# kharchenkolab/dropEst

Hardware: AMD Instinct MI355X
Metric: Mreads/s processed to final count matrix (higher is better)
Workload: dtype u64

## Files before the change

dropest_amd/csrc/context.h:

```cpp
#pragma once

#include <algorithm>
#include <chrono>
#include <condition_variable>
#include <functional>
#include <mutex>
#include <cstring>
#include <map>
#include <memory>
#include <string>
#include <thread>
#include <unordered_map>
#include <unordered_set>
#include <vector>

#include "../../include/dropest_amd.h"
#include "k_cbhash.h"
#include "k_collisions.h"
#include "k_merge.h"
#include "k_umi_directional.h"
#include "whitelist.h"
#include "k_misc.h"
#include "k_radix.h"
#include "k_ssort.h"
// ... 526 lines not shown
	u32 main_sort_passes = 0, main_sort_kind = 0;
	void scan_counts(const u32 *in, u32 *out, u32 n, u32 *total_out);
	dropest::DevBuf<u32> scan_chunk;
	void radix_sort(u64 *&keys, u32 *&vals, u64 *&keys_alt, u32 *&vals_alt, u32 n, u64 varying_mask, int val_bytes = 4,
	                const char *stat_prefix = nullptr);
	dropest::DevBuf<u64> ss_sample_a, ss_sample_b, ss_fine, ss_coarse;
	dropest::DevBuf<u32> ss_base1, ss_cnt2, ss_bucket_base, ss_bucket_cnt, ss_tmp, ss_n_loc, ss_prefix, ss_chunk, ss_big_list;
	struct RecvChunk { hipEvent_t ev; dropest::CbRanges rg; };
	std::vector<RecvChunk> recv_chunks;
	double hot_coverage = 0;
	dropest::DevBuf<u32> ss_cg_loc, ss_cg_cnt, ss_cg_prefix;
	bool cg_from_sort = false;
	dropest::DevBuf<u32> ss_cursors;
	bool ss_no_reserve = false;
	bool splitter_sort_reduce();
	void reduce_all();
	void reduce_molecules_to_cell_gene();
	void reduce_cell_gene_to_cells();
	void refresh_real_rows();
	void upload_whitelist();
	void search_merge_candidates(const std::vector<u32> &cells, const dropest::MergeUniverse &U, dropest::MergeSearch &S);
	void search_merge_candidates_host(const std::vector<u32> &cells, const dropest::MergeUniverse &U, dropest::MergeSearch &S);
	void build_merge_pairs(const std::vector<u32> &cells, dropest::MergeSearch &S);
	void decide_merge_targets(const dropest::MergeUniverse &U, dropest::MergeSearch &S, const std::vector<u32> &inter,
	                          std::vector<long> &targets, std::vector<u32> &target_ridx);
	std::vector<std::vector<u32>> replay_candidate_orders(const dropest::MergeUniverse &U, dropest::MergeSearch &S,
	                                                      const std::vector<u32> &need_order);
	std::vector<u32> pair_intersections(const std::vector<u32> &pair_base_cell, const std::vector<u32> &pair_cand_cell);
	void pair_intersections(const std::vector<u32> &pair_base_cell, const std::vector<u32> &pair_cand_cell, std::vector<u32> &inter);
	std::vector<double> poisson_expected_intersections(const std::vector<u32> &pair_base_cell, const std::vector<u32> &pair_cand_cell);
// ... 175 lines not shown
```

dropest_amd/csrc/dropest_amd.hip:

```cpp

#include "context.h"
extern "C" void dropest_bgzf_warm_up(void *stream);
#include "k_keyscatter.h"
#include "k_umidict.h"

#include <atomic>
#include <functional>
#include <map>
#include <mutex>

using namespace dropest;

static thread_local std::string g_last_error;

template <class F>
static dropest_status guarded(F &&f) {
	try {
		f();
		return DROPEST_OK;
	} catch (const InvalidError &e) { g_last_error = e.what(); return DROPEST_ERR_INVALID;
	} catch (const RangeError &e) { g_last_error = e.what(); return DROPEST_ERR_RANGE;
	} catch (const UnsupportedError &e) { g_last_error = e.what(); return DROPEST_ERR_UNSUPPORTED;
	} catch (const IoError &e) { g_last_error = e.what(); return DROPEST_ERR_IO;
	} catch (const DeviceError &e) { g_last_error = e.what(); return DROPEST_ERR_DEVICE;
// ... 885 lines not shown
	d_in.alloc(h.size()); d_out.alloc(h.size());
	HIP_CHECK(hipMemcpyAsync(d_in.p, h.data(), h.size() * 4, hipMemcpyHostToDevice, stream));
	hipLaunchKernelGGL(ss_lds_order_probe_kernel, dim3(1), dim3(64), 0, stream, d_in.p, rounds, d_out.p);
	HIP_CHECK(hipGetLastError());
	HIP_CHECK(hipMemcpyAsync(got.data(), d_out.p, got.size() * 4, hipMemcpyDeviceToHost, stream));
	HIP_CHECK(stream_wait(stream));
	bool ordered = true;
	for (u32 r = 0; r < rounds && ordered; ++r) {
		u32 seen[64] = {0};
		for (u32 l = 0; l < 64; ++l) { const u32 d = h[size_t(r) * 64 + l]; if (got[size_t(r) * 64 + l] != seen[d]) ordered = false; ++seen[d]; }
	}
	if (!ordered) fprintf(stderr, "[dropest_amd] device %d: LDS atomics of one instruction are not applied in lane order here; the finishing sort of the splitter sort ranks with ballots (slower, same results)\n", device);
	return known[device] = ordered;
}

bool dropest_ctx::splitter_sort_reduce() {
	const u32 n = u32(n_reads);
	const SsPlan plan = ss_plan(n_reads, chr_from_gene, layout.val_bytes);
	if (!plan.applicable) return false;
	const int tb = plan.tb, fb1 = plan.fb1, fb2 = plan.fb2;
	const bool wide = fb2 > 9;
	const u32 F1 = 1u << fb1, Ff = 1u << fb2, F2 = F1 * Ff;
	const int ms = layout.mark_shift, VB = layout.val_bytes;
	(void)tb;
	uint64_t os_max = plan.os;
	if (const char *e = getenv("DROPEST_SSORT_OS")) os_max = uint64_t(std::max(1, atoi(e)));
	const u32 os = u32(std::max<uint64_t>(1, std::min<uint64_t>(os_max, uint64_t(n) / (uint64_t(F2) * 2))));
	const u32 n_sample = F2 * os;
	const u64 order_mask = ~((1ull << ms) - 1ull);
	const u64 varying = (counters.key_or ^ counters.key_and) & order_mask;
// ... 11 lines not shown
	const int VB2 = rebase ? 0 : VB, ms2 = rebase ? 3 : ms;
	const u64 rebase_mask = rebase ? ~((1ull << layout.umi_bits) - 1ull) : 0ull;
	if (!in_l1) {
		ss_sample_a.ensure(n_sample); ss_sample_b.ensure(n_sample); ss_fine.ensure(F2); ss_coarse.ensure(F1);
		timed("ss_sample", double(n_sample) * 16, [&] {
			hipLaunchKernelGGL(ss_sample_kernel, dim3(div_up(n_sample, 256)), dim3(256), 0, stream, keys, n, ms, n_sample, ss_sample_a.p);
		});
		ss_splitters_from_sample(n_sample, os, Ff, F2, varying >> ms);
	}

	const u32 n_tiles = div_up(n, SS_TILE);
	u32 nblocks = std::min<u32>(n_tiles, 1024);
	const u32 tpb = div_up(n_tiles, nblocks);
	nblocks = div_up(n_tiles, tpb);
	const u32 parts = std::max<u32>(1, std::min<u32>(16, 2048 / F1));
	ss_bucket_base.ensure(F2); ss_bucket_cnt.ensure(F2); scalars.ensure(16);
	HIP_CHECK(hipMemsetAsync(scalars.p, 0, 16, stream));
	u32 max_cnt = 0;
	static const u32 SMALL_MAX = [] { const char *e = getenv("DROPEST_SS_SMALL_MAX"); return e && atoi(e) >= 256 && atoi(e) <= 2048 ? u32(atoi(e)) : 2048u; }();
	const bool atomic_rank = lds_atomics_lane_ordered(cfg.device, stream);
	ss_tmp.ensure(span * 2 + 2); ss_n_loc.ensure(F2); ss_prefix.ensure(F2); ss_chunk.ensure(1024);
	SsLocalArgs a{};
	a.keys = keys; a.vals = vals; a.bucket_base = ss_bucket_base.p; a.bucket_cnt = ss_bucket_cnt.p; a.n_buckets = F2; a.ms = ms2;
	if (rebase) { a.rebase_coarse = ss_coarse.p; a.rebase_mask = rebase_mask; a.rebase_div = Ff; }
	a.t_key = keys_alt; a.t_reads = ss_tmp.p; a.t_agg = ss_tmp.p + span; a.n_loc = ss_n_loc.p;
	if (const char *e = getenv("DROPEST_SS_DEBUG")) a.debug = u32(atoi(e));
	a.order_flag = scalars.p + 2;
	a.atomic_below = u32(ms2 + layout.umi_bits);
	if (const char *e = getenv("DROPEST_SS_ATOMIC_BELOW")) a.atomic_below = u32(atoi(e));
	a.cap = SMALL_MAX; a.skip_above = SMALL_MAX;
	const bool fused_cg_off = getenv("DROPEST_SS_NO_FUSED_CG") != nullptr;
	const bool fuse_cg = !fused_cg_off;
	cg_from_sort = false;
// ... 32 lines not shown
		if (!in_l1) timed(VB ? "ss_scatter:L1:key+1B" : "ss_scatter:L1:keys", double(n) * (8 + VB + 8 + VB2), [&] {
			auto go = [&](auto kernel) { hipLaunchKernelGGL(kernel, dim3(nblocks), dim3(SS_T), 0, stream, keys, vals, keys_alt, vals_alt, n, ms, fb1, ss_coarse.p, tpb, r1, rebase_mask); };
			if (rebase) { if (wide) go(ss_scatter_res_l1_kernel<1, 1024, true>); else if (fb1 <= 8 && !no256) go(ss_scatter_res_l1_kernel<1, 256, true>); else go(ss_scatter_res_l1_kernel<1, 512, true>); }
			else if (wide) { if (VB) go(ss_scatter_res_l1_kernel<1, 1024>); else go(ss_scatter_res_l1_kernel<0, 1024>); }
			else if (fb1 <= 8 && !no256) { if (VB) go(ss_scatter_res_l1_kernel<1, 256>); else go(ss_scatter_res_l1_kernel<0, 256>); }
			else { if (VB) go(ss_scatter_res_l1_kernel<1, 512>); else go(ss_scatter_res_l1_kernel<0, 512>); }
		});
		timed(VB2 ? "ss_scatter:L2:key+1B" : "ss_scatter:L2:keys", double(n) * 2 * (8 + VB2), [&] {
			auto go = [&](auto kernel) { hipLaunchKernelGGL(kernel, dim3(F1 * parts), dim3(SS_T), 0, stream, keys_alt, vals_alt, keys, vals, ms2, fb2, ss_fine.p, cur1, CS1, cap1, parts, r2,
			                                                 rebase ? ss_coarse.p : static_cast<const u64 *>(nullptr), rebase_mask); };
			if (wide) { if (VB2) go(ss_scatter_res_l2_kernel<1, 1024>); else go(ss_scatter_res_l2_kernel<0, 1024>); }
			else if (fb2 <= 8 && !no256) { if (VB2) go(ss_scatter_res_l2_kernel<1, 256>); else go(ss_scatter_res_l2_kernel<0, 256>); }
			else { if (VB2) go(ss_scatter_res_l2_kernel<1, 512>); else go(ss_scatter_res_l2_kernel<0, 512>); }
		});
		timed("ss_scan", double(F2) * 12, [&] {
			hipLaunchKernelGGL(ss_res_buckets_kernel, dim3(div_up(F2, 256)), dim3(256), 0, stream, cur2, F2, cap2, ss_bucket_base.p, ss_bucket_cnt.p, scalars.p);
		});
		launch_small();
		u32 head[4] = {0, 0, 0, 0};
		fetch(head, scalars.p, 16);
		max_cnt = head[0];
		if (head[3]) {
			stats["count:ss_reserve_overflow"].launches += 1;
			ss_no_reserve = true;
			build_keys(false);
			return splitter_sort_reduce();
		}
		if (max_cnt > SS_LOCAL_MAX) { build_keys(false, false); return false; }
	} else {
	rs_hist.ensure(size_t(F1) * nblocks); rs_row_total.ensure(1024); ss_base1.ensure(F1 + 1);
	timed("ss_hist:L1", double(n) * 8, [&] {
		if (wide) hipLaunchKernelGGL(ss_hist_l1_kernel<1024>, dim3(nblocks), dim3(SS_T), 0, stream, keys, n, ms, fb1, ss_coarse.p, tpb, rs_hist.p);
		else hipLaunchKernelGGL(ss_hist_l1_kernel<512>, dim3(nblocks), dim3(SS_T), 0, stream, keys, n, ms, fb1, ss_coarse.p, tpb, rs_hist.p);
	});
	timed("ss_scan", double(F1) * nblocks * 8, [&] {
		hipLaunchKernelGGL(rs_scan_rows_kernel, dim3(F1), dim3(256), 0, stream, rs_hist.p, nblocks, rs_row_total.p);
		if (wide) hipLaunchKernelGGL(ss_scan_totals_kernel<1024>, dim3(1), dim3(1024), 0, stream, rs_row_total.p, F1, n, ss_base1.p);
		else hipLaunchKernelGGL(ss_scan_totals_kernel<512>, dim3(1), dim3(512), 0, stream, rs_row_total.p, F1, n, ss_base1.p);
	});
	timed(VB ? "ss_scatter:L1:key+1B" : "ss_scatter:L1:keys", double(n) * 2 * (8 + VB), [&] {
		auto go = [&](auto kernel) { hipLaunchKernelGGL(kernel, dim3(nblocks), dim3(SS_T), 0, stream, keys, vals, keys_alt, vals_alt, n, ms, fb1, ss_coarse.p, tpb, rs_hist.p, ss_base1.p); };
		if (wide) { if (VB) go(ss_scatter_l1_kernel<1, 1024>); else go(ss_scatter_l1_kernel<0, 1024>); }
		else { if (VB) go(ss_scatter_l1_kernel<1, 512>); else go(ss_scatter_l1_kernel<0, 512>); }
	});

	ss_cnt2.ensure(size_t(F2) * parts);
	timed("ss_hist:L2", double(n) * 8, [&] {
		if (wide) hipLaunchKernelGGL(ss_hist_l2_kernel<1024>, dim3(F1 * parts), dim3(SS_T), 0, stream, keys_alt, ms, fb2, ss_fine.p, ss_base1.p, parts, ss_cnt2.p);
		else hipLaunchKernelGGL(ss_hist_l2_kernel<512>, dim3(F1 * parts), dim3(SS_T), 0, stream, keys_alt, ms, fb2, ss_fine.p, ss_base1.p, parts, ss_cnt2.p);
	});
	timed("ss_scan", double(F2) * parts * 8, [&] {
		if (wide) hipLaunchKernelGGL(ss_scan_seg_kernel<1024>, dim3(F1), dim3(1024), 0, stream, ss_cnt2.p, Ff, parts, ss_base1.p, ss_bucket_base.p, ss_bucket_cnt.p, scalars.p);
		else hipLaunchKernelGGL(ss_scan_seg_kernel<512>, dim3(F1), dim3(512), 0, stream, ss_cnt2.p, Ff, parts, ss_base1.p, ss_bucket_base.p, ss_bucket_cnt.p, scalars.p);
	});
	fetch(&max_cnt, scalars.p, 4);
	if (max_cnt > SS_LOCAL_MAX) return false;
	timed(VB ? "ss_scatter:L2:key+1B" : "ss_scatter:L2:keys", double(n) * 2 * (8 + VB), [&] {
		auto go = [&](auto kernel) { hipLaunchKernelGGL(kernel, dim3(F1 * parts), dim3(SS_T), 0, stream, keys_alt, vals_alt, keys, vals, ms, fb2, ss_fine.p, ss_base1.p, parts, ss_cnt2.p); };
		if (wide) { if (VB) go(ss_scatter_l2_kernel<1, 1024>); else go(ss_scatter_l2_kernel<0, 1024>); }
		else { if (VB) go(ss_scatter_l2_kernel<1, 512>); else go(ss_scatter_l2_kernel<0, 512>); }
	});
	}

	if (!reserve) launch_small();
	if (max_cnt > SMALL_MAX) {
		std::vector<u32> cnts(F2), medium, big;
		fetch(cnts.data(), ss_bucket_cnt.p, size_t(F2) * 4);
		for (u32 b = 0; b < F2; ++b) if (cnts[b] > SMALL_MAX) (cnts[b] <= 4096 ? medium : big).push_back(b);
		ss_big_list.ensure(medium.size() + big.size());
		if (!medium.empty()) HIP_CHECK(hipMemcpyAsync(ss_big_list.p, medium.data(), medium.size() * 4, hipMemcpyHostToDevice, stream));
		if (!big.empty()) HIP_CHECK(hipMemcpyAsync(ss_big_list.p + medium.size(), big.data(), big.size() * 4, hipMemcpyHostToDevice, stream));
		auto launch = [&](auto kernel, u32 threads, u32 cap, const u32 *list, size_t count) {
			SsLocalArgs g = a;
			g.big_list = list; g.cap = cap; g.skip_above = cap;
			const size_t lds = ss_local_lds_bytes(cap, int(threads));
			HIP_CHECK(hipFuncSetAttribute(reinterpret_cast<const void *>(kernel), hipFuncAttributeMaxDynamicSharedMemorySize, int(lds)));
			hipLaunchKernelGGL(kernel, dim3(u32(count)), dim3(threads), lds, stream, g);
		};
		timed("ss_local:big", 0, [&] {
			if (atomic_rank) {
				if (!medium.empty()) { if (VB2) launch(ss_local_big_kernel<256, 1, true>, 256, 4096, ss_big_list.p, medium.size()); else launch(ss_local_big_kernel<256, 0, true>, 256, 4096, ss_big_list.p, medium.size()); }
				if (!big.empty()) { if (VB2) launch(ss_local_big_kernel<512, 1, true>, 512, SS_LOCAL_MAX, ss_big_list.p + medium.size(), big.size()); else launch(ss_local_big_kernel<512, 0, true>, 512, SS_LOCAL_MAX, ss_big_list.p + medium.size(), big.size()); }
			} else {
				if (!medium.empty()) { if (VB2) launch(ss_local_big_kernel<256, 1>, 256, 4096, ss_big_list.p, medium.size()); else launch(ss_local_big_kernel<256, 0>, 256, 4096, ss_big_list.p, medium.size()); }
				if (!big.empty()) { if (VB2) launch(ss_local_big_kernel<512, 1>, 512, SS_LOCAL_MAX, ss_big_list.p + medium.size(), big.size()); else launch(ss_local_big_kernel<512, 0>, 512, SS_LOCAL_MAX, ss_big_list.p + medium.size(), big.size()); }
			}
		});
		HIP_CHECK(stream_wait(stream));
	}
	const u32 n_chunks = div_up(F2, 1024);
	timed("ss_scan", double(F2) * 12, [&] {
		hipLaunchKernelGGL(ss_chunk_sums_kernel<1024>, dim3(n_chunks), dim3(1024), 0, stream, ss_n_loc.p, F2, ss_chunk.p);
		hipLaunchKernelGGL(ss_prefix_kernel<1024>, dim3(n_chunks), dim3(1024), 0, stream, ss_n_loc.p, F2, ss_chunk.p, n_chunks, ss_prefix.p, scalars.p + 1);
		if (fuse_cg) {
			hipLaunchKernelGGL(ss_cg_counts_kernel, dim3(div_up(F2, 256)), dim3(256), 0, stream, ss_bucket_base.p, ss_n_loc.p, keys_alt, layout.umi_bits, F2, ss_cg_loc.p, ss_cg_cnt.p);
			hipLaunchKernelGGL(ss_chunk_sums_kernel<1024>, dim3(n_chunks), dim3(1024), 0, stream, ss_cg_cnt.p, F2, ss_chunk.p);
			hipLaunchKernelGGL(ss_prefix_kernel<1024>, dim3(n_chunks), dim3(1024), 0, stream, ss_cg_cnt.p, F2, ss_chunk.p, n_chunks, ss_cg_prefix.p, scalars.p + 4);
		}
	});
	u32 total_flag[4] = {0, 0, 0, 0};
	fetch(total_flag, scalars.p + 1, 16);
	if (total_flag[1]) {
		if (atomic_rank) lds_atomics_mark_unordered(cfg.device);
// ... 85 lines not shown
	const size_t quads = words / 4;
	for (uint32_t k = 0; k < a.n_arrays; ++k) {
		uint4 *q = reinterpret_cast<uint4 *>(a.p[k]);
		for (size_t i = size_t(blockIdx.x) * 256 + threadIdx.x; i < quads; i += size_t(gridDim.x) * 256) q[i] = make_uint4(0, 0, 0, 0);
		if (blockIdx.x == 0 && threadIdx.x < words - quads * 4) a.p[k][quads * 4 + threadIdx.x] = 0;
	}
}

void dropest_ctx::reduce_all() {
	const u32 n = u32(n_reads);
	u64 *keys = keys_a.p, *keys_alt = keys_b.p;
	u32 *vals = vals_a.p, *vals_alt = vals_b.p;
	const u64 order_mask = ~((1ull << layout.mark_shift) - 1ull);
	const u64 varying = (counters.key_or ^ counters.key_and) & order_mask;
	if (splitter_sort_reduce()) {
		n_chr_rows = 0;
		if (!cg_from_sort) reduce_molecules_to_cell_gene();
		reduce_cell_gene_to_cells();
		HIP_CHECK(stream_wait(stream));
		return;
	}
	main_sort_passes = u32(plan_radix_passes(varying).size()); main_sort_kind = 0;
	radix_sort(keys, vals, keys_alt, vals_alt, n, varying, layout.val_bytes);

	if (chr_from_gene) {
		auto run = [&](auto &p) {
			p.keys = keys;
			n_mol = run_segmented_reduce(*this, "molecules", p, n, 8 + layout.val_bytes, [&](u32 total) {
				mol_key.ensure(total + 1);
				for (DevBuf<u32> *b : {&mol_reads, &mol_mark, &mol_exon, &mol_intron}) b->ensure(total + 1);
// ... 1595 lines not shown
```

dropest_amd/csrc/k_misc.h:

```cpp
#pragma once

#include "k_cbhash.h"
#include "util.h"

namespace dropest {

__global__ __launch_bounds__(1024) void scan_small_kernel(const uint32_t *__restrict__ in, uint32_t *__restrict__ out,
                                                          uint32_t n, uint32_t *__restrict__ total_out) {
	__shared__ uint32_t scratch[1024 / 64 + 1];
	uint32_t carry = 0;
	for (uint32_t base = 0; base < n; base += 1024) {
		uint32_t i = base + threadIdx.x;
		uint32_t v = i < n ? in[i] : 0;
		uint32_t total;
		uint32_t ex = block_excl_scan_u32<1024>(v, scratch, total);
		if (i < n) out[i] = carry + ex;
		carry += total;
	}
	if (threadIdx.x == 0 && total_out) *total_out = carry;
}

struct KeyLayout {
	int umi_bits, gene_bits, cell_bits;
	int mark_shift;
// ... 292 lines not shown
				}
				if (t < total - tail0) { a.t_drow8[out + tail0 + t] = stage_d[tail0 + t]; a.t_val8[out + tail0 + t] = stage_v[tail0 + t]; }
			}
			if (threadIdx.x == 0 && total) kept_row[0] = kept_row[total];
		} else if (keep) {
			if (NARROW) {
				a.t_gene16[out + ex] = uint16_t(g);
				a.t_val16[out + ex] = v >= 0xFFFFu ? uint16_t(0xFFFFu) : uint16_t(v);
				if (v >= 0xFFFFu) {
					const uint32_t at = atomicAdd(a.ovf_count, 1u);
					if (at < a.ovf_cap) { a.ovf_pos[at] = out + ex; a.ovf_val[at] = v; }
				}
			} else { a.t_gene[out + ex] = g; a.t_val[out + ex] = v; }
		}
		out += total;
	}
}

constexpr uint32_t EMS_COLS = 8, EMS_STAGE = EMS_COLS * 255u;
__global__ __launch_bounds__(256) void emit_matrix_bytes_short_kernel(MatrixArgs a) {
	__shared__ uint32_t st_pos[2][EMS_STAGE], st_val[2][EMS_STAGE];
	__shared__ uint32_t st_n[2], st_base[2];
	const uint32_t lane = threadIdx.x & 63u, w = threadIdx.x >> 6;
	if (threadIdx.x < 2) st_n[threadIdx.x] = 0;
	__syncthreads();
	for (uint32_t c = w; c < EMS_COLS; c += 4) {
		const uint32_t idx = blockIdx.x * EMS_COLS + c;
		if (idx >= a.n_list) break;
		const uint32_t col = a.col_list[idx];
		const uint32_t cell = a.col_cell[col];
// ... 453 lines not shown
```

dropest_amd/csrc/k_ssort.h:

```cpp
#pragma once

#include "util.h"

namespace dropest {

constexpr int SS_T = 512, SS_I = 8, SS_TILE = SS_T * SS_I;
constexpr int SS_MAX_F = 512;
constexpr uint32_t SS_LOCAL_MAX = 8192;

__global__ __launch_bounds__(256) void ss_sample_kernel(const unsigned long long *__restrict__ keys, uint32_t n, int ms,
                                                        uint32_t n_sample, unsigned long long *__restrict__ out) {
	const uint32_t j = blockIdx.x * 256 + threadIdx.x;
	if (j >= n_sample) return;
	const uint32_t pos = uint32_t((uint64_t(j) * n + n / 2) / n_sample);
	out[j] = keys[pos < n ? pos : n - 1] >> ms;
}

__global__ __launch_bounds__(256) void ss_pick_splitters_kernel(const unsigned long long *__restrict__ sorted_sample, uint32_t os, uint32_t F, uint32_t F2,
                                                                unsigned long long *__restrict__ fine, unsigned long long *__restrict__ coarse) {
	const uint32_t j = blockIdx.x * 256 + threadIdx.x;
	if (j >= F2) return;
	const unsigned long long v = j + 1 < F2 ? sorted_sample[size_t(j + 1) * os] : ~0ull;
	fine[j] = v;
	if ((j + 1) % F == 0) coarse[(j + 1) / F - 1] = v;
// ... 65 lines not shown
__global__ __launch_bounds__(SS_T) void ss_hist_l2_kernel(const unsigned long long *__restrict__ keys, int ms, int fb,
                                                          const unsigned long long *__restrict__ fine, const uint32_t *__restrict__ base1,
                                                          uint32_t parts, uint32_t *__restrict__ cnt2) {
	__shared__ unsigned long long sp[MAXF];
	__shared__ uint32_t cnt[MAXF];
	const uint32_t F = 1u << fb, s = blockIdx.x / parts, p = blockIdx.x % parts;
	for (uint32_t j = threadIdx.x; j < F; j += SS_T) { sp[j] = j + 1 < F ? fine[size_t(s) * F + j] : ~0ull; cnt[j] = 0; }
	__syncthreads();
	uint32_t begin, end;
	ss_l2_range(base1, s, p, parts, begin, end);
	if (begin < end) ss_hist_range(keys, begin, end, ms, fb, sp, cnt);
	__syncthreads();
	for (uint32_t j = threadIdx.x; j < F; j += SS_T) cnt2[(size_t(s) * F + j) * parts + p] = cnt[j];
}

template <int MAXF>
__global__ __launch_bounds__(MAXF) void ss_scan_seg_kernel(uint32_t *__restrict__ cnt2, uint32_t F, uint32_t parts,
                                                            const uint32_t *__restrict__ base1, uint32_t *__restrict__ bucket_base,
                                                            uint32_t *__restrict__ bucket_cnt, uint32_t *__restrict__ max_cnt) {
	__shared__ uint32_t scratch[MAXF / 64 + 1];
	const uint32_t s = blockIdx.x, f = threadIdx.x;
	uint32_t *row = cnt2 + (size_t(s) * F + f) * parts;
	uint32_t sum = 0;
	if (f < F) for (uint32_t p = 0; p < parts; ++p) sum += row[p];
	uint32_t total;
	const uint32_t ex = block_excl_scan_u32<MAXF>(sum, scratch, total);
	if (f < F) {
		uint32_t run = base1[s] + ex;
		bucket_base[size_t(s) * F + f] = run;
		bucket_cnt[size_t(s) * F + f] = sum;
		for (uint32_t p = 0; p < parts; ++p) { const uint32_t c = row[p]; row[p] = run; run += c; }
	}
	const unsigned long long m = wave_reduce_max_u64(sum);
	if (lane_id() == 0 && m) atomicMax(max_cnt, uint32_t(m));
}

template <int VB, int MAXF>
__device__ inline void ss_scatter_range(const unsigned long long *__restrict__ keys, const uint8_t *__restrict__ vals,
                                        unsigned long long *__restrict__ okeys, uint8_t *__restrict__ ovals, uint32_t begin, uint32_t end,
                                        int ms, int fb, const unsigned long long *sp, uint32_t *goff, uint32_t *cnt, uint32_t *tstart,
                                        uint32_t *gdelta, uint32_t *scratch, unsigned long long *sk, uint16_t *sd, uint8_t *sv) {
	constexpr int PER = MAXF / SS_T;
	const uint32_t F = 1u << fb, tid = threadIdx.x;
	for (uint32_t t0 = begin; t0 < end; t0 += SS_TILE) {
		const uint32_t in_tile = end - t0 < uint32_t(SS_TILE) ? end - t0 : uint32_t(SS_TILE);
		for (uint32_t j = tid; j < F; j += SS_T) cnt[j] = 0;
		lds_barrier();
		unsigned long long key[SS_I];
		uint8_t val[VB ? SS_I : 1];
// ... 225 lines not shown
	const unsigned long long lo = (rebase_coarse && s) ? (rebase_coarse[s - 1] & rebase_mask) : 0ull;
	for (uint32_t j = threadIdx.x; j < F; j += SS_T) {
		const unsigned long long f = j + 1 < F ? fine[size_t(s) * F + j] : ~0ull;
		sp[j] = j + 1 < F ? (f > lo ? f - lo : 0ull) : ~0ull;
	}
	__syncthreads();
	const uint32_t fill = cur1[size_t(s) * cstride1], sb = s * cap1, se = sb + (fill < cap1 ? fill : cap1);
	const uint32_t tiles = (se - sb + SS_TILE - 1) / SS_TILE, tpp = (tiles + parts - 1) / parts;
	const uint64_t b = uint64_t(sb) + uint64_t(p) * tpp * SS_TILE, e = b + uint64_t(tpp) * SS_TILE;
	const uint32_t begin = b < se ? uint32_t(b) : se, end = e < se ? uint32_t(e) : se;
	SsReserve mine = rs;
	mine.first = s * F;
	if (begin < end) ss_scatter_res_range<VB, MAXF>(keys, vals, okeys, ovals, begin, end, ms, fb, sp, mine, cnt, tstart, gdelta, scratch, sk, sd, sv);
}
__global__ __launch_bounds__(256) void ss_res_buckets_kernel(const uint32_t *__restrict__ cur2, uint32_t n_buckets, uint32_t cap,
                                                             uint32_t *__restrict__ bucket_base, uint32_t *__restrict__ bucket_cnt, uint32_t *__restrict__ max_cnt) {
	const uint32_t b = blockIdx.x * 256 + threadIdx.x;
	uint32_t c = 0;
	if (b < n_buckets) { c = cur2[b] < cap ? cur2[b] : cap; bucket_base[b] = b * cap; bucket_cnt[b] = c; }
	const unsigned long long m = wave_reduce_max_u64(c);
	if (lane_id() == 0 && m) atomicMax(max_cnt, uint32_t(m));
}

struct SsLocalArgs {
	const unsigned long long *keys;
	const uint8_t *vals;
	const uint32_t *bucket_base, *bucket_cnt;
	const uint32_t *big_list;
	uint32_t n_buckets;
	int ms;
	uint32_t cap;
	uint32_t skip_above;
	uint32_t debug;
	uint32_t atomic_below;
	uint32_t *order_flag;
	unsigned long long *t_key;
	uint32_t *t_reads, *t_agg, *n_loc;
	uint32_t *cg_loc;
	int cg_shift;
	const unsigned long long *rebase_coarse;
	unsigned long long rebase_mask;
	uint32_t rebase_div;
};

template <int THREADS, int ITEMS, int VB, bool ATOMIC_RANK = false>
__device__ inline void ss_local_run(const SsLocalArgs &a, uint32_t bucket, uint32_t base, uint32_t cnt, unsigned char *smem) {
	constexpr uint32_t WAVES = THREADS / 64;
	const uint32_t tid = threadIdx.x, w = tid >> 6, lane = tid & 63u;
	unsigned long long *sk = reinterpret_cast<unsigned long long *>(smem);
	uint32_t *agg = reinterpret_cast<uint32_t *>(smem);
	uint32_t *headpos = agg + a.cap;
	uint32_t *wcnt = reinterpret_cast<uint32_t *>(smem + size_t(a.cap) * 8);
	uint32_t *tstart = wcnt + WAVES * 256;
	uint32_t *scratch = tstart + 256;
	uint32_t *wtot = scratch + (THREADS / 64 + 1);
	uint32_t *misc = wtot + WAVES;
	unsigned long long *red = reinterpret_cast<unsigned long long *>(misc + 4 + ((WAVES + 1) & 1u));
	uint8_t *sv = reinterpret_cast<uint8_t *>(red + 2 * WAVES);
	const int ms = a.ms;
	const uint32_t coarse_b = a.rebase_coarse ? bucket / a.rebase_div : 0u;
	const unsigned long long kbase = coarse_b ? (a.rebase_coarse[coarse_b - 1u] & a.rebase_mask) : 0ull;

	const uint32_t lane_off = w * (64 * ITEMS) + lane;
	unsigned long long key[ITEMS];
	uint8_t val[VB ? ITEMS : 1];
	unsigned long long k_or = 0, k_and = ~0ull;
#pragma unroll
	for (int i = 0; i < ITEMS; ++i) {
		const uint32_t p = lane_off + i * 64;
		const bool valid = p < cnt;
		key[i] = valid ? a.keys[base + p] : 0ull;
		if (VB) val[i] = valid ? a.vals[base + p] : uint8_t(0);
	}
#pragma unroll
	for (int i = 0; i < ITEMS; ++i) {
		const uint32_t p = lane_off + i * 64;
		if (p < cnt) { k_or |= key[i]; k_and &= key[i]; sk[p] = key[i]; if (VB) sv[p] = val[i]; }
	}
	k_or = wave_reduce_or_u64(k_or); k_and = wave_reduce_and_u64(k_and);
	if (lane == 0) { red[2 * w] = k_or; red[2 * w + 1] = k_and; }
	lds_barrier();
	k_or = 0; k_and = ~0ull;
#pragma unroll
	for (uint32_t k = 0; k < WAVES; ++k) { k_or |= red[2 * k]; k_and &= red[2 * k + 1]; }
	const unsigned long long vary = (k_or ^ k_and) & ~((1ull << ms) - 1ull);

	for (int shift = vary ? __builtin_ctzll(vary) : 64; shift < 64 && (vary >> shift) != 0; shift += 8) {
		if (((vary >> shift) & 0xFFull) == 0 || (a.debug & 2u)) continue;
		for (uint32_t j = tid; j < WAVES * 256; j += THREADS) wcnt[j] = 0;
		lds_barrier();
		uint32_t lrank[ITEMS];
		const bool by_atomic = ATOMIC_RANK && uint32_t(shift) < a.atomic_below;
		const uint32_t vbits = uint32_t(vary >> shift) & 0xFFu;
#pragma unroll
		for (int i = 0; i < ITEMS; ++i) {
			const bool valid = (lane_off + i * 64) < cnt;
			const uint32_t d = uint32_t(key[i] >> shift) & 0xFFu;
			if (by_atomic) { lrank[i] = valid ? atomicAdd(&wcnt[w * 256 + d], 1u) : 0u; continue; }
			uint32_t diff_lo = 0, diff_hi = 0;
			for (uint32_t left = vbits; left; left &= left - 1u) {
				const int b = __builtin_ctz(left);
				const int32_t mine = int32_t(d << (31 - b)) >> 31;
				const unsigned long long bal = __ballot(mine != 0);
				diff_lo |= uint32_t(bal) ^ uint32_t(mine);
				diff_hi |= uint32_t(bal >> 32) ^ uint32_t(mine);
			}
			unsigned long long m = ~(((unsigned long long)diff_hi << 32) | diff_lo);
			m &= __ballot(valid);
			const uint32_t before = __builtin_amdgcn_mbcnt_hi(uint32_t(m >> 32), __builtin_amdgcn_mbcnt_lo(uint32_t(m), 0u));
			const uint32_t old = wcnt[w * 256 + d];
// ... 19 lines not shown
			for (uint32_t j = 0; j < PER; ++j) {
				const uint32_t d = tid * PER + j;
				uint32_t run = 0;
#pragma unroll
				for (uint32_t k = 0; k < WAVES; ++k) { const uint32_t c = wcnt[k * 256 + d]; wcnt[k * 256 + d] = run; run += c; }
				tot[j] = run; sum += run;
			}
			uint32_t total;
			uint32_t ex = block_excl_scan_u32<THREADS, true>(sum, scratch, total);
#pragma unroll
			for (uint32_t j = 0; j < PER; ++j) { tstart[tid * PER + j] = ex; ex += tot[j]; }
		}
		lds_barrier();
#pragma unroll
		for (int i = 0; i < ITEMS; ++i)
			if ((lane_off + i * 64) < cnt) {
				const uint32_t d = uint32_t(key[i] >> shift) & 0xFFu;
				const uint32_t q = tstart[d] + wcnt[w * 256 + d] + lrank[i];
				sk[q] = key[i];
				if (VB) sv[q] = val[i];
			}
		lds_barrier();
#pragma unroll
		for (int i = 0; i < ITEMS; ++i) {
			const uint32_t p = lane_off + i * 64;
			if (p < cnt) { key[i] = sk[p]; if (VB) val[i] = sv[p]; }
		}
	}

	uint32_t run = 0, pre[ITEMS], head_bits = 0, cg_heads = 0;
	bool out_of_order = false;
#pragma unroll
	for (int i = 0; i < ITEMS; ++i) {
		const uint32_t p = lane_off + i * 64;
		const bool valid = p < cnt;
		const unsigned long long prev = (valid && p) ? sk[p - 1] : 0ull;
		out_of_order |= valid && p && (prev >> ms) > (key[i] >> ms);
		const bool head = valid && (p == 0 || (prev >> ms) != (key[i] >> ms));
		const unsigned long long bal = __ballot(head);
		pre[i] = run + __builtin_amdgcn_mbcnt_hi(uint32_t(bal >> 32), __builtin_amdgcn_mbcnt_lo(uint32_t(bal), 0u));
		run += uint32_t(__popcll(bal));
		if (head) head_bits |= 1u << i;
		if (a.cg_loc) cg_heads += uint32_t(__popcll(__ballot(valid && p && (prev >> a.cg_shift) != (key[i] >> a.cg_shift))));
	}
	if (lane == 0) wtot[w] = run;
	if (a.cg_loc && lane == 0 && cg_heads) atomicAdd(&a.cg_loc[bucket], cg_heads);
	if (__ballot(out_of_order) && lane == 0) atomicOr(a.order_flag, 1u);
	lds_barrier();
	uint32_t woff = 0, n_loc = 0;
#pragma unroll
	for (uint32_t k = 0; k < WAVES; ++k) { const uint32_t t = wtot[k]; if (k < w) woff += t; n_loc += t; }
	for (uint32_t m = tid; m < n_loc; m += THREADS) agg[m] = 0;
	if (tid == 0) a.n_loc[bucket] = n_loc;
	lds_barrier();
#pragma unroll
	for (int i = 0; i < ITEMS; ++i) {
		const uint32_t p = lane_off + i * 64;
		if (p >= cnt) continue;
		const uint32_t is_head = (head_bits >> i) & 1u;
		const uint32_t m = woff + pre[i] + is_head - 1u;
		const uint32_t mark = VB ? uint32_t(val[i]) & 7u : uint32_t(key[i]) & 7u;
		if (is_head) { headpos[m] = p; a.t_key[base + m] = (key[i] >> ms) + kbase; }
		const uint32_t add = (((mark >> 1) & 1u) << 1) | (((mark >> 2) & 1u) << 16);
		if (add) atomicAdd(&agg[m], add);
		if (mark & 1u) atomicOr(&agg[m], 1u);
	}
	lds_barrier();
	for (uint32_t m = tid; m < n_loc; m += THREADS) {
		const uint32_t e = m + 1 < n_loc ? headpos[m + 1] : cnt;
		a.t_reads[base + m] = e - headpos[m];
		a.t_agg[base + m] = agg[m];
	}
}

template <int VB, bool ATOMIC_RANK = false>
__global__ __launch_bounds__(256) void ss_local_kernel(SsLocalArgs a) {
	extern __shared__ __attribute__((aligned(16))) unsigned char ss_smem[];
	const uint32_t b = blockIdx.x;
	const uint32_t cnt = a.bucket_cnt[b], base = a.bucket_base[b];
	if (cnt == 0) { if (threadIdx.x == 0) a.n_loc[b] = 0; return; }
	if (cnt > a.skip_above) return;
	if (cnt <= 1024) ss_local_run<256, 4, VB, ATOMIC_RANK>(a, b, base, cnt, ss_smem);
	else ss_local_run<256, 8, VB, ATOMIC_RANK>(a, b, base, cnt, ss_smem);
}
template <int THREADS, int VB, bool ATOMIC_RANK = false>
__global__ __launch_bounds__(THREADS) void ss_local_wave_kernel(SsLocalArgs a) {
	extern __shared__ __attribute__((aligned(16))) unsigned char ss_smem[];
	const uint32_t b = blockIdx.x;
	const uint32_t cnt = a.bucket_cnt[b], base = a.bucket_base[b];
	if (cnt == 0) { if (threadIdx.x == 0) a.n_loc[b] = 0; return; }
	if (cnt > a.skip_above) return;
	if (cnt <= 1024) ss_local_run<THREADS, 1024 / THREADS, VB, ATOMIC_RANK>(a, b, base, cnt, ss_smem);
	else ss_local_run<THREADS, 2048 / THREADS, VB, ATOMIC_RANK>(a, b, base, cnt, ss_smem);
}
template <int THREADS, int VB, bool ATOMIC_RANK = false>
__global__ __launch_bounds__(THREADS) void ss_local_big_kernel(SsLocalArgs a) {
	extern __shared__ __attribute__((aligned(16))) unsigned char ss_smem[];
	const uint32_t b = a.big_list[blockIdx.x];
// ... 255 lines not shown
```

dropest_amd/csrc/matrix_emit.h:

```cpp
#pragma once

#include <sys/syscall.h>
#include <unistd.h>

static u32 checked_nnz(uint64_t nnz) {
	if (nnz > 0xFFFFFFF0ull) throw UnsupportedError("count matrix with more than 2^32 non-zeros");
	return u32(nnz);
}

void dropest_ctx::matrix_columns(bool filtered_m, std::vector<u32> &col_cell, std::vector<u32> &colptr, uint64_t &nnz) {
	col_cell.clear(); colptr.clear();
	nnz = 0;
	if (filtered_m) {
		filtered_cells();
		for (u32 ri : filtered_ridx) {
			const HostCell &h = real[ri];
			col_cell.push_back(h.id); colptr.push_back(u32(nnz)); nnz += h.row.requested_genes;
		}
	} else {
		constexpr unsigned W = dropest::HostPool::MAX;
		size_t cols[W] = {0}; uint64_t sums[W] = {0};
		auto is_col = [&](const HostCell &h) { return !(h.merged || h.excluded || h.row.n_genes < min_before); };
		const unsigned workers = parallel_ranges(real.size(), [&](size_t b, size_t e, unsigned w) {
			size_t c = 0; uint64_t s = 0;
// ... 58 lines not shown
}

void dropest_ctx::launch_emit(int dev_form, dropest::MatrixArgs a, MatrixResult &M, hipStream_t st) {
	using namespace dropest;
	const u32 ncols = u32(M.ncols);
	if (dev_form == 0) { hipLaunchKernelGGL(emit_matrix_kernel<0>, dim3(ncols), dim3(256), 0, st, a); return; }
	if (dev_form == 1) { hipLaunchKernelGGL(emit_matrix_kernel<1>, dim3(ncols), dim3(256), 0, st, a); return; }
	auto is_long = [&](u32 j) { return M.colptr[j + 1] - M.colptr[j] >= 256u; };
	M.col_list_host.resize(ncols);
	u32 n_long = 0;
	for (u32 j = 0; j < ncols; ++j) if (is_long(j)) M.col_list_host[n_long++] = j;
	u32 at = n_long;
	for (u32 j = 0; j < ncols; ++j) if (!is_long(j)) M.col_list_host[at++] = j;
	M.d_col_list.ensure(ncols);
	HIP_CHECK(hipMemcpyAsync(M.d_col_list.p, M.col_list_host.data(), size_t(ncols) * 4, hipMemcpyHostToDevice, st));
	if (n_long) { a.col_list = M.d_col_list.p; a.n_list = n_long; hipLaunchKernelGGL(emit_matrix_kernel<2>, dim3(n_long), dim3(256), 0, st, a); }
	if (ncols > n_long) {
		a.col_list = M.d_col_list.p + n_long; a.n_list = ncols - n_long;
		hipLaunchKernelGGL(emit_matrix_bytes_short_kernel, dim3(div_up(a.n_list, EMS_COLS)), dim3(256), 0, st, a);
	}
}

void dropest_ctx::matrix_copy_out(MatrixResult &M, uint64_t nnz, hipStream_t st) {
	if (M.narrow == 2) {
		HIP_CHECK(hipMemcpyAsync(M.h_drow8.p, M.d_drow8.p, nnz, hipMemcpyDeviceToHost, st));
		HIP_CHECK(hipMemcpyAsync(M.h_val8.p, M.d_val8.p, nnz, hipMemcpyDeviceToHost, st));
		HIP_CHECK(hipMemcpyAsync(M.vals.h_count(), M.vals.d_count(), 4, hipMemcpyDeviceToHost, st));
		HIP_CHECK(hipMemcpyAsync(M.rows.h_count(), M.rows.d_count(), 4, hipMemcpyDeviceToHost, st));
	} else if (M.narrow == 1) {
		HIP_CHECK(hipMemcpyAsync(M.h_row16.p, M.d_row16.p, nnz * 2, hipMemcpyDeviceToHost, st));
		HIP_CHECK(hipMemcpyAsync(M.h_val16.p, M.d_val16.p, nnz * 2, hipMemcpyDeviceToHost, st));
// ... 522 lines not shown
```

Baseline: 11200.

## Build oversize bucket lists on device, size local sort per bucket, add byte emit kernel

The scan kernels now classify oversize buckets into medium and big lists on the device with wave ballots and an atomic counter. This replaces the host fetch of all bucket counts, the host partitioning, the list upload and a stream wait. The local sort picks exact items-per-thread variants (5, 6, 7 or 8) and skips unused register slots when fewer items are needed. A new raw byte-packed emit kernel writes four delta and value bytes per thread for long columns when zeros are not skipped. Extra profiling statistics are added, and list ordering now depends on atomics, so the order of bucket processing may differ between runs.

```diff
diff --git a/dropest_amd/csrc/context.h b/dropest_amd/csrc/context.h
--- a/dropest_amd/csrc/context.h
+++ b/dropest_amd/csrc/context.h
@@ -564,6 +564,8 @@
 	dropest::DevBuf<u32> ss_cursors;
 	bool ss_no_reserve = false;
 	bool splitter_sort_reduce();
+	u32 ss_stat_buckets = 0, ss_stat_small_max = 0;
+	void ss_count_items_per_wave(u32 F2, u32 small_max);
 	void reduce_all();
 	void reduce_molecules_to_cell_gene();
 	void reduce_cell_gene_to_cells();
diff --git a/dropest_amd/csrc/dropest_amd.hip b/dropest_amd/csrc/dropest_amd.hip
--- a/dropest_amd/csrc/dropest_amd.hip
+++ b/dropest_amd/csrc/dropest_amd.hip
@@ -923,6 +923,14 @@
 	return known[device] = ordered;
 }
 
+void dropest_ctx::ss_count_items_per_wave(u32 F2, u32 small_max) {
+	std::vector<u32> cnts(F2);
+	fetch(cnts.data(), ss_bucket_cnt.p, size_t(F2) * 4);
+	u32 by_ipw[17] = {0};
+	for (u32 c : cnts) if (c && c <= SS_LOCAL_MAX) by_ipw[div_up(c, c <= small_max || c <= 4096u ? 256u : 512u)] += 1;
+	for (u32 k = 1; k <= 16; ++k) if (by_ipw[k]) stats["count:ss_local_ipw" + std::to_string(k)].launches += by_ipw[k];
+}
+
 bool dropest_ctx::splitter_sort_reduce() {
 	const u32 n = u32(n_reads);
 	const SsPlan plan = ss_plan(n_reads, chr_from_gene, layout.val_bytes);
@@ -964,9 +972,10 @@
 	const u32 tpb = div_up(n_tiles, nblocks);
 	nblocks = div_up(n_tiles, tpb);
 	const u32 parts = std::max<u32>(1, std::min<u32>(16, 2048 / F1));
-	ss_bucket_base.ensure(F2); ss_bucket_cnt.ensure(F2); scalars.ensure(16);
-	HIP_CHECK(hipMemsetAsync(scalars.p, 0, 16, stream));
-	u32 max_cnt = 0;
+	ss_bucket_base.ensure(F2); ss_bucket_cnt.ensure(F2); ss_big_list.ensure(F2); scalars.ensure(16);
+	HIP_CHECK(hipMemsetAsync(scalars.p, 0, 32, stream));
+	u32 max_cnt = 0, n_medium = 0, n_big = 0;
+	unsigned long long *const big_counts = reinterpret_cast<unsigned long long *>(scalars.p + 6);
 	static const u32 SMALL_MAX = [] { const char *e = getenv("DROPEST_SS_SMALL_MAX"); return e && atoi(e) >= 256 && atoi(e) <= 2048 ? u32(atoi(e)) : 2048u; }();
 	const bool atomic_rank = lds_atomics_lane_ordered(cfg.device, stream);
 	ss_tmp.ensure(span * 2 + 2); ss_n_loc.ensure(F2); ss_prefix.ensure(F2); ss_chunk.ensure(1024);
@@ -1029,12 +1038,13 @@
 			else { if (VB2) go(ss_scatter_res_l2_kernel<1, 512>); else go(ss_scatter_res_l2_kernel<0, 512>); }
 		});
 		timed("ss_scan", double(F2) * 12, [&] {
-			hipLaunchKernelGGL(ss_res_buckets_kernel, dim3(div_up(F2, 256)), dim3(256), 0, stream, cur2, F2, cap2, ss_bucket_base.p, ss_bucket_cnt.p, scalars.p);
+			hipLaunchKernelGGL(ss_res_buckets_kernel, dim3(div_up(F2, 256)), dim3(256), 0, stream, cur2, F2, cap2, ss_bucket_base.p, ss_bucket_cnt.p, scalars.p,
+			                   SMALL_MAX, ss_big_list.p, big_counts);
 		});
 		launch_small();
-		u32 head[4] = {0, 0, 0, 0};
-		fetch(head, scalars.p, 16);
-		max_cnt = head[0];
+		u32 head[8] = {0, 0, 0, 0, 0, 0, 0, 0};
+		fetch(head, scalars.p, 32);
+		max_cnt = head[0]; n_medium = head[6]; n_big = head[7];
 		if (head[3]) {
 			stats["count:ss_reserve_overflow"].launches += 1;
 			ss_no_reserve = true;
@@ -1065,10 +1075,14 @@
 		else hipLaunchKernelGGL(ss_hist_l2_kernel<512>, dim3(F1 * parts), dim3(SS_T), 0, stream, keys_alt, ms, fb2, ss_fine.p, ss_base1.p, parts, ss_cnt2.p);
 	});
 	timed("ss_scan", double(F2) * parts * 8, [&] {
-		if (wide) hipLaunchKernelGGL(ss_scan_seg_kernel<1024>, dim3(F1), dim3(1024), 0, stream, ss_cnt2.p, Ff, parts, ss_base1.p, ss_bucket_base.p, ss_bucket_cnt.p, scalars.p);
-		else hipLaunchKernelGGL(ss_scan_seg_kernel<512>, dim3(F1), dim3(512), 0, stream, ss_cnt2.p, Ff, parts, ss_base1.p, ss_bucket_base.p, ss_bucket_cnt.p, scalars.p);
-	});
-	fetch(&max_cnt, scalars.p, 4);
+		if (wide) hipLaunchKernelGGL(ss_scan_seg_kernel<1024>, dim3(F1), dim3(1024), 0, stream, ss_cnt2.p, Ff, parts, ss_base1.p, ss_bucket_base.p, ss_bucket_cnt.p, scalars.p, SMALL_MAX, ss_big_list.p, big_counts);
+		else hipLaunchKernelGGL(ss_scan_seg_kernel<512>, dim3(F1), dim3(512), 0, stream, ss_cnt2.p, Ff, parts, ss_base1.p, ss_bucket_base.p, ss_bucket_cnt.p, scalars.p, SMALL_MAX, ss_big_list.p, big_counts);
+	});
+	{
+		u32 head[8] = {0, 0, 0, 0, 0, 0, 0, 0};
+		fetch(head, scalars.p, 32);
+		max_cnt = head[0]; n_medium = head[6]; n_big = head[7];
+	}
 	if (max_cnt > SS_LOCAL_MAX) return false;
 	timed(VB ? "ss_scatter:L2:key+1B" : "ss_scatter:L2:keys", double(n) * 2 * (8 + VB), [&] {
 		auto go = [&](auto kernel) { hipLaunchKernelGGL(kernel, dim3(F1 * parts), dim3(SS_T), 0, stream, keys_alt, vals_alt, keys, vals, ms, fb2, ss_fine.p, ss_base1.p, parts, ss_cnt2.p); };
@@ -1078,13 +1092,10 @@
 	}
 
 	if (!reserve) launch_small();
+	ss_stat_buckets = F2; ss_stat_small_max = SMALL_MAX;
 	if (max_cnt > SMALL_MAX) {
-		std::vector<u32> cnts(F2), medium, big;
-		fetch(cnts.data(), ss_bucket_cnt.p, size_t(F2) * 4);
-		for (u32 b = 0; b < F2; ++b) if (cnts[b] > SMALL_MAX) (cnts[b] <= 4096 ? medium : big).push_back(b);
-		ss_big_list.ensure(medium.size() + big.size());
-		if (!medium.empty()) HIP_CHECK(hipMemcpyAsync(ss_big_list.p, medium.data(), medium.size() * 4, hipMemcpyHostToDevice, stream));
-		if (!big.empty()) HIP_CHECK(hipMemcpyAsync(ss_big_list.p + medium.size(), big.data(), big.size() * 4, hipMemcpyHostToDevice, stream));
+		const u32 *const medium_list = ss_big_list.p, *const big_list = ss_big_list.p + (F2 - n_big);
+		if (profiling) { stats["count:ss_local_medium_buckets"].launches += n_medium; stats["count:ss_local_big_buckets"].launches += n_big; }
 		auto launch = [&](auto kernel, u32 threads, u32 cap, const u32 *list, size_t count) {
 			SsLocalArgs g = a;
 			g.big_list = list; g.cap = cap; g.skip_above = cap;
@@ -1094,14 +1105,13 @@
 		};
 		timed("ss_local:big", 0, [&] {
 			if (atomic_rank) {
-				if (!medium.empty()) { if (VB2) launch(ss_local_big_kernel<256, 1, true>, 256, 4096, ss_big_list.p, medium.size()); else launch(ss_local_big_kernel<256, 0, true>, 256, 4096, ss_big_list.p, medium.size()); }
-				if (!big.empty()) { if (VB2) launch(ss_local_big_kernel<512, 1, true>, 512, SS_LOCAL_MAX, ss_big_list.p + medium.size(), big.size()); else launch(ss_local_big_kernel<512, 0, true>, 512, SS_LOCAL_MAX, ss_big_list.p + medium.size(), big.size()); }
+				if (n_medium) { if (VB2) launch(ss_local_big_kernel<256, 1, true>, 256, 4096, medium_list, n_medium); else launch(ss_local_big_kernel<256, 0, true>, 256, 4096, medium_list, n_medium); }
+				if (n_big) { if (VB2) launch(ss_local_big_kernel<512, 1, true>, 512, SS_LOCAL_MAX, big_list, n_big); else launch(ss_local_big_kernel<512, 0, true>, 512, SS_LOCAL_MAX, big_list, n_big); }
 			} else {
-				if (!medium.empty()) { if (VB2) launch(ss_local_big_kernel<256, 1>, 256, 4096, ss_big_list.p, medium.size()); else launch(ss_local_big_kernel<256, 0>, 256, 4096, ss_big_list.p, medium.size()); }
-				if (!big.empty()) { if (VB2) launch(ss_local_big_kernel<512, 1>, 512, SS_LOCAL_MAX, ss_big_list.p + medium.size(), big.size()); else launch(ss_local_big_kernel<512, 0>, 512, SS_LOCAL_MAX, ss_big_list.p + medium.size(), big.size()); }
+				if (n_medium) { if (VB2) launch(ss_local_big_kernel<256, 1>, 256, 4096, medium_list, n_medium); else launch(ss_local_big_kernel<256, 0>, 256, 4096, medium_list, n_medium); }
+				if (n_big) { if (VB2) launch(ss_local_big_kernel<512, 1>, 512, SS_LOCAL_MAX, big_list, n_big); else launch(ss_local_big_kernel<512, 0>, 512, SS_LOCAL_MAX, big_list, n_big); }
 			}
 		});
-		HIP_CHECK(stream_wait(stream));
 	}
 	const u32 n_chunks = div_up(F2, 1024);
 	timed("ss_scan", double(F2) * 12, [&] {
@@ -1217,6 +1227,7 @@
 	const u64 order_mask = ~((1ull << layout.mark_shift) - 1ull);
 	const u64 varying = (counters.key_or ^ counters.key_and) & order_mask;
 	if (splitter_sort_reduce()) {
+		if (profiling) ss_count_items_per_wave(ss_stat_buckets, ss_stat_small_max);
 		n_chr_rows = 0;
 		if (!cg_from_sort) reduce_molecules_to_cell_gene();
 		reduce_cell_gene_to_cells();
diff --git a/dropest_amd/csrc/k_misc.h b/dropest_amd/csrc/k_misc.h
--- a/dropest_amd/csrc/k_misc.h
+++ b/dropest_amd/csrc/k_misc.h
@@ -330,6 +330,55 @@
 			} else { a.t_gene[out + ex] = g; a.t_val[out + ex] = v; }
 		}
 		out += total;
+	}
+}
+
+__global__ __launch_bounds__(256) void emit_matrix_bytes_raw_kernel(MatrixArgs a) {
+	const uint32_t col = a.col_list ? a.col_list[blockIdx.x] : blockIdx.x;
+	const uint32_t cell = a.col_cell[col];
+	const uint32_t b = a.cell_cg_begin[cell], rows = a.cell_cg_count[cell];
+	if (rows == 0) return;
+	const uint32_t len = rows - ((a.cg_key[b + rows - 1u] & a.gene_mask) == a.gene_mask ? 1u : 0u);
+	const uint32_t out = a.col_start[col];
+	auto entry = [&](bool on, uint32_t k, uint32_t prev1, uint32_t g, uint32_t v, uint32_t &db, uint32_t &vb) {
+		const uint32_t delta = g + 1u - prev1;
+		db = delta >= 255u ? 255u : delta;
+		vb = v >= 255u ? 255u : v;
+		matrix_list_append(on && delta >= 255u, out + k, g, a.rovf_count, a.rovf_pos, a.rovf_row, a.rovf_cap);
+		matrix_list_append(on && v >= 255u, out + k, v, a.ovf_count, a.ovf_pos, a.ovf_val, a.ovf_cap);
+	};
+	const uint32_t head = min(len, (4u - (out & 3u)) & 3u), nw = (len - head) >> 2, tail0 = head + 4u * nw, t = threadIdx.x;
+	if (t < 64u) {
+		const bool front = t < head, back = t >= 3u && t - 3u < len - tail0;
+		const uint32_t k = front ? t : tail0 + (t - 3u);
+		uint32_t g = 0, v = 0, prev1 = 0, db, vb;
+		if (front || back) {
+			g = uint32_t(a.cg_key[b + k] & a.gene_mask); v = a.value[b + k];
+			if (k) prev1 = uint32_t(a.cg_key[b + k - 1u] & a.gene_mask) + 1u;
+		}
+		entry(front || back, k, prev1, g, v, db, vb);
+		if (front || back) { a.t_drow8[out + k] = uint8_t(db); a.t_val8[out + k] = uint8_t(vb); }
+	}
+	for (uint32_t w0 = 0; w0 < nw; w0 += 256u) {
+		const uint32_t wi = w0 + t;
+		const bool on = wi < nw;
+		const uint32_t k0 = head + 4u * wi;
+		uint32_t g[4] = {0, 0, 0, 0}, v[4] = {0, 0, 0, 0}, prev1 = 0, dword = 0, vword = 0;
+		if (on) {
+			if (k0) prev1 = uint32_t(a.cg_key[b + k0 - 1u] & a.gene_mask) + 1u;
+#pragma unroll
+			for (uint32_t j = 0; j < 4; ++j) { g[j] = uint32_t(a.cg_key[b + k0 + j] & a.gene_mask); v[j] = a.value[b + k0 + j]; }
+		}
+#pragma unroll
+		for (uint32_t j = 0; j < 4; ++j) {
+			uint32_t db, vb;
+			entry(on, k0 + j, j ? g[j - 1] + 1u : prev1, g[j], v[j], db, vb);
+			dword |= db << (8u * j); vword |= vb << (8u * j);
+		}
+		if (on) {
+			*reinterpret_cast<uint32_t *>(a.t_drow8 + out + k0) = dword;
+			*reinterpret_cast<uint32_t *>(a.t_val8 + out + k0) = vword;
+		}
 	}
 }
 
diff --git a/dropest_amd/csrc/k_ssort.h b/dropest_amd/csrc/k_ssort.h
--- a/dropest_amd/csrc/k_ssort.h
+++ b/dropest_amd/csrc/k_ssort.h
@@ -103,10 +103,25 @@
 	for (uint32_t j = threadIdx.x; j < F; j += SS_T) cnt2[(size_t(s) * F + j) * parts + p] = cnt[j];
 }
 
+__device__ inline void ss_list_oversize(uint32_t c, uint32_t bucket, uint32_t small_max, uint32_t n_buckets, uint32_t *__restrict__ list,
+                                        unsigned long long *__restrict__ counts) {
+	const bool medium = c > small_max && c <= 4096u, big = c > small_max && c > 4096u;
+	const unsigned long long mm = __ballot(medium), mb = __ballot(big);
+	if (!(mm | mb)) return;
+	const uint32_t lane = lane_id(), first = uint32_t(__builtin_ctzll(mm | mb));
+	unsigned long long old = 0;
+	if (lane == first) old = atomicAdd(counts, (unsigned long long)__popcll(mm) | ((unsigned long long)__popcll(mb) << 32));
+	const uint32_t old_m = uint32_t(__shfl(int(uint32_t(old)), int(first), 64)), old_b = uint32_t(__shfl(int(uint32_t(old >> 32)), int(first), 64));
+	const unsigned long long below = (1ull << lane) - 1ull;
+	if (medium) list[old_m + uint32_t(__popcll(mm & below))] = bucket;
+	if (big) list[n_buckets - 1u - (old_b + uint32_t(__popcll(mb & below)))] = bucket;
+}
+
 template <int MAXF>
 __global__ __launch_bounds__(MAXF) void ss_scan_seg_kernel(uint32_t *__restrict__ cnt2, uint32_t F, uint32_t parts,
                                                             const uint32_t *__restrict__ base1, uint32_t *__restrict__ bucket_base,
-                                                            uint32_t *__restrict__ bucket_cnt, uint32_t *__restrict__ max_cnt) {
+                                                            uint32_t *__restrict__ bucket_cnt, uint32_t *__restrict__ max_cnt,
+                                                            uint32_t small_max, uint32_t *__restrict__ big_list, unsigned long long *__restrict__ big_counts) {
 	__shared__ uint32_t scratch[MAXF / 64 + 1];
 	const uint32_t s = blockIdx.x, f = threadIdx.x;
 	uint32_t *row = cnt2 + (size_t(s) * F + f) * parts;
@@ -122,6 +137,7 @@
 	}
 	const unsigned long long m = wave_reduce_max_u64(sum);
 	if (lane_id() == 0 && m) atomicMax(max_cnt, uint32_t(m));
+	ss_list_oversize(f < F ? sum : 0u, s * F + f, small_max, gridDim.x * F, big_list, big_counts);
 }
 
 template <int VB, int MAXF>
@@ -377,12 +393,14 @@
 	if (begin < end) ss_scatter_res_range<VB, MAXF>(keys, vals, okeys, ovals, begin, end, ms, fb, sp, mine, cnt, tstart, gdelta, scratch, sk, sd, sv);
 }
 __global__ __launch_bounds__(256) void ss_res_buckets_kernel(const uint32_t *__restrict__ cur2, uint32_t n_buckets, uint32_t cap,
-                                                             uint32_t *__restrict__ bucket_base, uint32_t *__restrict__ bucket_cnt, uint32_t *__restrict__ max_cnt) {
+                                                             uint32_t *__restrict__ bucket_base, uint32_t *__restrict__ bucket_cnt, uint32_t *__restrict__ max_cnt,
+                                                             uint32_t small_max, uint32_t *__restrict__ big_list, unsigned long long *__restrict__ big_counts) {
 	const uint32_t b = blockIdx.x * 256 + threadIdx.x;
 	uint32_t c = 0;
 	if (b < n_buckets) { c = cur2[b] < cap ? cur2[b] : cap; bucket_base[b] = b * cap; bucket_cnt[b] = c; }
 	const unsigned long long m = wave_reduce_max_u64(c);
 	if (lane_id() == 0 && m) atomicMax(max_cnt, uint32_t(m));
+	ss_list_oversize(c, b, small_max, n_buckets, big_list, big_counts);
 }
 
 struct SsLocalArgs {
@@ -406,7 +424,7 @@
 	uint32_t rebase_div;
 };
 
-template <int THREADS, int ITEMS, int VB, bool ATOMIC_RANK = false>
+template <int THREADS, int ITEMS, int VB, bool ATOMIC_RANK = false, bool EXACT = false>
 __device__ inline void ss_local_run(const SsLocalArgs &a, uint32_t bucket, uint32_t base, uint32_t cnt, unsigned char *smem) {
 	constexpr uint32_t WAVES = THREADS / 64;
 	const uint32_t tid = threadIdx.x, w = tid >> 6, lane = tid & 63u;
@@ -424,12 +442,14 @@
 	const uint32_t coarse_b = a.rebase_coarse ? bucket / a.rebase_div : 0u;
 	const unsigned long long kbase = coarse_b ? (a.rebase_coarse[coarse_b - 1u] & a.rebase_mask) : 0ull;
 
-	const uint32_t lane_off = w * (64 * ITEMS) + lane;
+	const uint32_t ipw = EXACT ? uint32_t(ITEMS) : (cnt + THREADS - 1) / THREADS;
+	const uint32_t lane_off = w * (64 * ipw) + lane;
 	unsigned long long key[ITEMS];
 	uint8_t val[VB ? ITEMS : 1];
 	unsigned long long k_or = 0, k_and = ~0ull;
 #pragma unroll
 	for (int i = 0; i < ITEMS; ++i) {
+		if (uint32_t(i) >= ipw) continue;
 		const uint32_t p = lane_off + i * 64;
 		const bool valid = p < cnt;
 		key[i] = valid ? a.keys[base + p] : 0ull;
@@ -437,6 +457,7 @@
 	}
 #pragma unroll
 	for (int i = 0; i < ITEMS; ++i) {
+		if (uint32_t(i) >= ipw) continue;
 		const uint32_t p = lane_off + i * 64;
 		if (p < cnt) { k_or |= key[i]; k_and &= key[i]; sk[p] = key[i]; if (VB) sv[p] = val[i]; }
 	}
@@ -457,6 +478,7 @@
 		const uint32_t vbits = uint32_t(vary >> shift) & 0xFFu;
 #pragma unroll
 		for (int i = 0; i < ITEMS; ++i) {
+			if (uint32_t(i) >= ipw) continue;
 			const bool valid = (lane_off + i * 64) < cnt;
 			const uint32_t d = uint32_t(key[i] >> shift) & 0xFFu;
 			if (by_atomic) { lrank[i] = valid ? atomicAdd(&wcnt[w * 256 + d], 1u) : 0u; continue; }
@@ -506,7 +528,7 @@
 		lds_barrier();
 #pragma unroll
 		for (int i = 0; i < ITEMS; ++i)
-			if ((lane_off + i * 64) < cnt) {
+			if (uint32_t(i) < ipw && (lane_off + i * 64) < cnt) {
 				const uint32_t d = uint32_t(key[i] >> shift) & 0xFFu;
 				const uint32_t q = tstart[d] + wcnt[w * 256 + d] + lrank[i];
 				sk[q] = key[i];
@@ -515,6 +537,7 @@
 		lds_barrier();
 #pragma unroll
 		for (int i = 0; i < ITEMS; ++i) {
+			if (uint32_t(i) >= ipw) continue;
 			const uint32_t p = lane_off + i * 64;
 			if (p < cnt) { key[i] = sk[p]; if (VB) val[i] = sv[p]; }
 		}
@@ -524,6 +547,7 @@
 	bool out_of_order = false;
 #pragma unroll
 	for (int i = 0; i < ITEMS; ++i) {
+		if (uint32_t(i) >= ipw) continue;
 		const uint32_t p = lane_off + i * 64;
 		const bool valid = p < cnt;
 		const unsigned long long prev = (valid && p) ? sk[p - 1] : 0ull;
@@ -547,6 +571,7 @@
 	lds_barrier();
 #pragma unroll
 	for (int i = 0; i < ITEMS; ++i) {
+		if (uint32_t(i) >= ipw) continue;
 		const uint32_t p = lane_off + i * 64;
 		if (p >= cnt) continue;
 		const uint32_t is_head = (head_bits >> i) & 1u;
@@ -573,7 +598,10 @@
 	if (cnt == 0) { if (threadIdx.x == 0) a.n_loc[b] = 0; return; }
 	if (cnt > a.skip_above) return;
 	if (cnt <= 1024) ss_local_run<256, 4, VB, ATOMIC_RANK>(a, b, base, cnt, ss_smem);
-	else ss_local_run<256, 8, VB, ATOMIC_RANK>(a, b, base, cnt, ss_smem);
+	else if (cnt <= 1280) ss_local_run<256, 5, VB, ATOMIC_RANK, true>(a, b, base, cnt, ss_smem);
+	else if (cnt <= 1536) ss_local_run<256, 6, VB, ATOMIC_RANK, true>(a, b, base, cnt, ss_smem);
+	else if (cnt <= 1792) ss_local_run<256, 7, VB, ATOMIC_RANK, true>(a, b, base, cnt, ss_smem);
+	else ss_local_run<256, 8, VB, ATOMIC_RANK, true>(a, b, base, cnt, ss_smem);
 }
 template <int THREADS, int VB, bool ATOMIC_RANK = false>
 __global__ __launch_bounds__(THREADS) void ss_local_wave_kernel(SsLocalArgs a) {
diff --git a/dropest_amd/csrc/matrix_emit.h b/dropest_amd/csrc/matrix_emit.h
--- a/dropest_amd/csrc/matrix_emit.h
+++ b/dropest_amd/csrc/matrix_emit.h
@@ -96,7 +96,11 @@
 	for (u32 j = 0; j < ncols; ++j) if (!is_long(j)) M.col_list_host[at++] = j;
 	M.d_col_list.ensure(ncols);
 	HIP_CHECK(hipMemcpyAsync(M.d_col_list.p, M.col_list_host.data(), size_t(ncols) * 4, hipMemcpyHostToDevice, st));
-	if (n_long) { a.col_list = M.d_col_list.p; a.n_list = n_long; hipLaunchKernelGGL(emit_matrix_kernel<2>, dim3(n_long), dim3(256), 0, st, a); }
+	if (n_long) {
+		a.col_list = M.d_col_list.p; a.n_list = n_long;
+		if (!a.skip_zero) hipLaunchKernelGGL(emit_matrix_bytes_raw_kernel, dim3(n_long), dim3(256), 0, st, a);
+		else hipLaunchKernelGGL(emit_matrix_kernel<2>, dim3(n_long), dim3(256), 0, st, a);
+	}
 	if (ncols > n_long) {
 		a.col_list = M.d_col_list.p + n_long; a.n_list = ncols - n_long;
 		hipLaunchKernelGGL(emit_matrix_bytes_short_kernel, dim3(div_up(a.n_list, EMS_COLS)), dim3(256), 0, st, a);
```

Result: slower. 11000 (-1.8%).
